# Ignalina/znippy

Measured on AMD Instinct MI355X. Metric: decompress MB/s (uncompressed) + compress MB/s, 100k x 10KB archive, higher is better.
Workload: dtype u8; 1 GPU; 100k x 10KiB text chunks (BASELINE configs[1]); rows_per_gpu=100000, chunk_bytes=10240, bytes_per_gpu=1024000000, blob_bytes_per_gpu=6400000, parallelism=row-cursor ranges x1, pipelining=step k+1 queued before step k's counters are read (two runs in flight)

## Files before the change

znippy_amd/csrc/api.hip:

```cpp
#include <unistd.h>
#include "common.h"
#include "encode.h"
#include "../../include/znippy_hip.h"

#include <algorithm>
#include <cstdio>
#include <cstdlib>
#include <cstring>
#include <chrono>
#include <memory>
#include <new>
#include <stdexcept>
#include <string>
#include <vector>
#include <unordered_map>

namespace zn {
int measure_b3_pass_ns(int cus, hipStream_t s, float *ns_per_pass_per_simd, float *ghz);
size_t decode_lit_scratch_bytes(int grid);
void set_fused_dbg(unsigned long long *p);
void set_fused_abl(int v);
}

using namespace zn;
// ... 63 lines not shown
    uint64_t bx_fse_cap = 0, bx_huf_cap = 0;
    uint32_t *rx_pool = nullptr, *rx_chunk = nullptr;
    uint8_t *rx_cdone = nullptr;
    uint64_t rx_cap = 0;
    uint8_t *vs_pool = nullptr;
    uint64_t vs_cap = 0;
    uint8_t *rr_pool[2] = {nullptr, nullptr};
    uint64_t rr_cap[2] = {0, 0};
    hipEvent_t ev_fork = nullptr, ev_join = nullptr, ev_join2 = nullptr;
    std::vector<KTime> ktimes;
    int n_ktimes = 0;
    std::vector<hipEvent_t> event_pool;
    bool ktime_open = false;
    std::vector<std::pair<size_t, void *>> pinned_pool;
    size_t pinned_pool_bytes = 0;
    std::vector<std::pair<size_t, void *>> dev_pool;
    std::unordered_map<void *, size_t> dev_sizes;
    size_t dev_pool_bytes = 0;
    struct {
        int dbg = 0;
        unsigned lds_pad = 0;
        int store_g = 0;
        bool no_block_items = false, no_fused_blocks = false, ddbg = false, edbg = false, no_fused_store = false,
             nohash = false, no_roles = false, no_fz = false, fz_only = false, no_bx = false, tdbg = false, no_fuse_hash = false, trace = false, no_rx = false, no_pack = false, no_lean = false, no_stored_only = false;
        unsigned roles_min = 2048;
        unsigned bx_big = BX_BIG_SEQ;
        bool bx_big_set = false;
        int ktime = 2;
    } sw;
    int cus = 256;
    int live_tables = 0;
    bool closing = false;
    unsigned long long *clk_buf = nullptr;
    enum Diag { DIAG_FUSED, DIAG_ITEMS, DIAG_FZ, DIAG_GENERAL, DIAG_BX, DIAG_ENCODE, DIAG_N };
    unsigned long long *diag[DIAG_N] = {};
};

static void read_switches(znippy_ctx *ctx) {
    auto on = [](const char *n) { const char *v = getenv(n); return v && *v && *v != '0'; };
    if (const char *e = getenv("ZNIPPY_DBG")) ctx->sw.dbg = atoi(e);
    if (const char *e = getenv("ZNIPPY_LDS_PAD")) ctx->sw.lds_pad = (unsigned)atoi(e);
    ctx->sw.no_block_items = on("ZNIPPY_NO_BLOCK_ITEMS");
    ctx->sw.no_fused_blocks = on("ZNIPPY_NO_FUSED_BLOCKS");
    ctx->sw.ddbg = on("ZNIPPY_DDBG");
    ctx->sw.edbg = on("ZNIPPY_EDBG");
    ctx->sw.no_fused_store = on("ZNIPPY_NO_FUSED_STORE");
    ctx->sw.nohash = on("ZNIPPY_NOHASH");
    ctx->sw.no_roles = on("ZNIPPY_NO_ROLES");
    ctx->sw.no_fz = on("ZNIPPY_NO_FZ");
    ctx->sw.tdbg = on("ZNIPPY_TDBG");
    ctx->sw.trace = on("ZNIPPY_TRACE");
    ctx->sw.no_lean = on("ZNIPPY_NO_LEAN");
    ctx->sw.no_pack = on("ZNIPPY_NO_PACK");
    if (const char *e = getenv("ZNIPPY_STORE_G")) ctx->sw.store_g = atoi(e) == 1 ? 1 : (atoi(e) == 2 ? 2 : 0);
    ctx->sw.no_stored_only = on("ZNIPPY_NO_STORED_ONLY");
    ctx->sw.no_rx = on("ZNIPPY_NO_RX");
    ctx->sw.no_fuse_hash = on("ZNIPPY_NO_FUSE_HASH");
    ctx->sw.no_bx = on("ZNIPPY_NO_BX");
    if (const char *e = getenv("ZNIPPY_BX_BIG")) { ctx->sw.bx_big = (unsigned)atoi(e); ctx->sw.bx_big_set = true; }
    if (const char *lv = getenv("ZNIPPY_LEVEL")) { const int v = atoi(lv); if (v >= 1 && v <= 22) ctx->level = v; }
    if (const char *wl = getenv("ZNIPPY_WINDOW_LOG")) { const int v = atoi(wl); if (v == 0 || (v >= WINDOW_LOG_MIN && v <= WINDOW_LOG_MAX)) ctx->window_log = v; }
    if (const char *gs = getenv("ZNIPPY_GEN_SHARE")) { const int v = atoi(gs); if (v >= 1 && v <= 4) ctx->gen_share = v; }
    ctx->sw.fz_only = on("ZNIPPY_FZ_ONLY");
    if (const char *e = getenv("ZNIPPY_ROLES_MIN")) ctx->sw.roles_min = (unsigned)atoi(e);
    if (const char *e = getenv("ZNIPPY_KTIME")) ctx->sw.ktime = atoi(e);
}

static void *pinned_take(znippy_ctx *ctx, size_t bytes, size_t *cap) {
    size_t best = ctx->pinned_pool.size();
    for (size_t i = 0; i < ctx->pinned_pool.size(); i++)
        if (ctx->pinned_pool[i].first >= bytes && ctx->pinned_pool[i].first <= 4 * bytes + 4096 &&
            (best == ctx->pinned_pool.size() || ctx->pinned_pool[i].first < ctx->pinned_pool[best].first))
            best = i;
    if (best != ctx->pinned_pool.size()) {
        void *p = ctx->pinned_pool[best].second;
// ... 187 lines not shown
static_assert(ctl_before(CTL_COUNTERS, CTL_HAND) && ctl_before(CTL_HAND, CTL_CURSORS) && ctl_before(CTL_CURSORS, CTL_FZ_POOL) && ctl_before(CTL_FZ_POOL, CTL_BX_POOL) &&
              ctl_before(CTL_BX_POOL, CTL_BX_CTR) && ctl_before(CTL_BX_CTR, CTL_RX) && CTL_RX.at + CTL_RX.bytes <= CTL_HEAD, "control block: regions overlap or pass the head");
static_assert(CTL_COUNTERS.at == 0 && CTL_HAND.at == CTL_COUNTERS.bytes && CTL_MIRROR == CTL_HAND.at + CTL_HAND.bytes, "the mirror is exactly counters + hand-over counts");
static_assert(CTL_FLAG < 8 && H_FLAGGED == H_SERIAL + 4 && H_FLAGGED < 8 && CUR_FZ_WORK < 16 && zn::RX_ROUNDS <= RX_ZERO && RX_ZERO < 16, "control block: a word outside its region");

struct znippy_rows {
    znippy_ctx *ctx = nullptr;
    uint64_t row_begin = 0;
    uint32_t n = 0;
    uint32_t n_compressed = 0;
    uint64_t *blob_off = nullptr, *blob_size = nullptr, *usize = nullptr, *out_off = nullptr;
    uint8_t *compressed = nullptr, *checksum = nullptr, *d_bitmap = nullptr;
    uint32_t *h_pack = nullptr, *d_pack = nullptr;
    size_t h_pack_cap = 0;
    unsigned long long *d_pack_sums = nullptr;
    uint8_t *ctl = nullptr;
    size_t ctl_bytes = 0;
    template <class T> T *ctl_at(CtlRegion g, size_t i = 0) const { return reinterpret_cast<T *>(ctl + g.at) + i; }
    uint32_t *hand(Hand h) const { return ctl_at<uint32_t>(CTL_HAND, h); }
    uint32_t *cur(Cursor c) const { return ctl_at<uint32_t>(CTL_CURSORS, c); }
    int32_t *status = nullptr;
    uint32_t *digests = nullptr;
    uint64_t *counters = nullptr;
    uint64_t *h_counters = nullptr;
    const uint32_t *mirror_hand(unsigned slot) const { return reinterpret_cast<const uint32_t *>(reinterpret_cast<const uint8_t *>(h_counters + 16 * slot) + CTL_HAND.at); }
    size_t h_counters_cap = 0;
    int bx_hint = -1;
    bool lean_ok = false;
    int lean_hint = -1;
    bool lean_blocks_ok = false;
    bool lean_mixed_ok = false;
    bool roles_off = false;
    bool small_ok = false, small_off = false;
    uint32_t *all_rows = nullptr;
    int lean_hint2 = -1;
    int plain_hint = -1;
    struct RunArgs { const void *blobs = nullptr; void *out = nullptr; uint64_t base = 0, cap = 0, blob_cap = ~0ull; bool verify = false, plain = false; } run_args[2];
    uint64_t *vs_off = nullptr;
    uint64_t vs_bytes = 0;
    bool vs_built = false;
    bool no_out = false;
    hipEvent_t ev_done[2] = {nullptr, nullptr};
    uint64_t run_seq = 0;
    uint64_t ext_min_bo = 0, ext_max_bend = 0, ext_max_oend = 0;
    bool ext_wrap = false;
    std::vector<uint64_t> h_blob_off, h_blob_size, h_len, h_out_off;
// ... 457 lines not shown
        ctx->own_stream = true;
    }
    init_fused_tables();
    if (hipStreamCreateWithFlags(&ctx->aux, hipStreamNonBlocking) != hipSuccess ||
        hipStreamCreateWithFlags(&ctx->copy, hipStreamNonBlocking) != hipSuccess ||
        hipEventCreateWithFlags(&ctx->ev_fork, hipEventDisableTiming) != hipSuccess ||
        hipEventCreateWithFlags(&ctx->ev_join, hipEventDisableTiming) != hipSuccess ||
        hipEventCreateWithFlags(&ctx->ev_join2, hipEventDisableTiming) != hipSuccess) {
        znippy_ctx_destroy(ctx);
        return ZNIPPY_E_HIP;
    }
    ctx->decode_grid = decode_grid_size(device);
    if (hipMalloc(&ctx->cursor, 64) != hipSuccess) {
        znippy_ctx_destroy(ctx);
        return ZNIPPY_E_NOMEM;
    }
    {
        hipDeviceProp_t p;
        int cus = hipGetDeviceProperties(&p, device) == hipSuccess ? p.multiProcessorCount : 256;
        ctx->cus = cus;
        ctx->encode_grid = cus * 8;
        ctx->encode_grid_small = cus * 16;
    }
    *out = ctx;
    return ZNIPPY_OK;
}

static void ctx_teardown(znippy_ctx *ctx);
void znippy_ctx_destroy(znippy_ctx *ctx) {
    if (!ctx || ctx->closing) return;
    if (ctx->live_tables) {
        (void)hipSetDevice(ctx->device);
        (void)hipStreamSynchronize(ctx->stream);
        ctx->closing = true;
        return;
    }
    ctx_teardown(ctx);
}
static void table_released(znippy_ctx *ctx) {
    if (--ctx->live_tables == 0 && ctx->closing) ctx_teardown(ctx);
}
static void ctx_teardown(znippy_ctx *ctx) {
    (void)hipSetDevice(ctx->device);
    (void)hipStreamSynchronize(ctx->stream);
    for (auto &k : ctx->ktimes) { (void)hipEventDestroy(k.t0); (void)hipEventDestroy(k.t1); }
    void *dev[] = {ctx->lit_scratch, ctx->lit_scratch_b, ctx->fz_lit_pool, ctx->fz_seq_pool, ctx->bx_fse_pool, ctx->bx_huf_pool, ctx->rx_pool, ctx->rx_chunk, ctx->rx_cdone, ctx->cursor, ctx->vs_pool, ctx->rr_pool[0], ctx->rr_pool[1],
                   ctx->clk_buf, ctx->shim_in, ctx->shim_out, ctx->enc_prov, ctx->enc_seq, ctx->enc_tabs, ctx->ldm};
    for (void *p : dev) if (p) (void)hipFree(p);
    for (unsigned long long *d : ctx->diag) if (d) (void)hipFree(d);
    if (ctx->aux) { (void)hipStreamSynchronize(ctx->aux); (void)hipStreamDestroy(ctx->aux); }
    if (ctx->copy) { (void)hipStreamSynchronize(ctx->copy); (void)hipStreamDestroy(ctx->copy); }
    for (auto &e : ctx->pinned_pool) (void)hipHostFree(e.second);
    for (auto &e : ctx->dev_pool) (void)hipFree(e.second);
    for (hipEvent_t e : ctx->event_pool) (void)hipEventDestroy(e);
    if (ctx->ev_fork) (void)hipEventDestroy(ctx->ev_fork);
    if (ctx->ev_join) (void)hipEventDestroy(ctx->ev_join);
    if (ctx->ev_join2) (void)hipEventDestroy(ctx->ev_join2);
    if (ctx->own_stream) (void)hipStreamDestroy(ctx->stream);
    delete ctx;
}

const char *znippy_last_error(const znippy_ctx *ctx) { return ctx ? ctx->err.c_str() : "null context"; }

int znippy_ctx_sync(znippy_ctx *ctx) {
    if (ctx && ctx->closing) return ZNIPPY_E_INVAL;
    if (!ctx) return ZNIPPY_E_INVAL;
    HIPCHK(ctx, hipStreamSynchronize(ctx->stream));
    if (ctx->copy) HIPCHK(ctx, hipStreamSynchronize(ctx->copy));
    return ZNIPPY_OK;
}

int znippy_last_kernel_times(znippy_ctx *ctx, const char **names, float *ms, int cap) {
    if (ctx && ctx->closing) return ZNIPPY_E_INVAL;
    if (!ctx) return 0;
    int n = std::min(cap, ctx->n_ktimes);
    for (int i = 0; i < n; i++) {
        names[i] = ctx->ktimes[i].name;
        ms[i] = 0.f;
        (void)hipEventElapsedTime(&ms[i], ctx->ktimes[i].t0, ctx->ktimes[i].t1);
    }
    return n;
}

int znippy_rows_foreign_stats(znippy_ctx *ctx, znippy_rows *r, uint64_t stats[8]) {
    if (ctx && ctx->closing) return ZNIPPY_E_INVAL;
    if (!ctx || !r || r->ctx != ctx || !stats) return ZNIPPY_E_INVAL;
    HIPCHK(ctx, hipSetDevice(ctx->device));
    HIPCHK(ctx, hipStreamSynchronize(ctx->stream));
    HIPCHK(ctx, hipMemcpy(stats, r->ctl + (r->bx_slots ? CTL_BX_POOL : CTL_FZ_POOL).at, 64, hipMemcpyDeviceToHost));
    return ZNIPPY_OK;
// ... 69 lines not shown
    if (n < 5) return ZNIPPY_E_CORRUPT;
    uint32_t magic;
    memcpy(&magic, p, 4);
    if (magic != 0xFD2FB528u) return ZNIPPY_E_CORRUPT;
    uint32_t fhd = p[4], fcs_flag = fhd >> 6, single = (fhd >> 5) & 1, did_flag = fhd & 3;
    if (fhd & 8) return ZNIPPY_E_CORRUPT;
    uint32_t fcs_bytes = fcs_flag == 0 ? single : (1u << fcs_flag);
    uint32_t did_bytes = did_flag == 3 ? 4 : did_flag;
    size_t pos = 5 + (single ? 0 : 1) + did_bytes;
    if (n < pos + fcs_bytes) return ZNIPPY_E_CORRUPT;
    if (!fcs_bytes) return ZNIPPY_E_UNSUPPORTED;
    uint64_t fcs = 0;
    for (uint32_t i = 0; i < fcs_bytes; i++) fcs |= (uint64_t)p[pos + i] << (8 * i);
    if (fcs_bytes == 2) fcs += 256;
    *out_size = fcs;
    return ZNIPPY_OK;
}


void znippy_rows_destroy(znippy_rows *r) {
    if (!r) return;
    (void)hipSetDevice(r->ctx->device);
    void *ptrs[] = {r->blob_off, r->blob_size, r->usize, r->out_off, r->compressed, r->checksum,
                    r->ctl, r->digests, r->corrupt, r->list_a, r->pending,
                    r->cand_row, r->cand_base, r->cand_nblocks, r->fz_base, r->fz_cap, r->fz_it_cand, r->fz_nb, r->fz_work, r->fz_items, r->item_row, r->item_k, r->item_src, r->row_flag, r->pending2,
                    r->bt_tile, r->bt_item, r->tile_done, r->todo, r->status_init, r->slow_list,
                    r->bx_cand_row, r->bx_cand_base, r->bx_cand_nb, r->bx_huf_list, r->bx_seq_list, r->bx_items, r->bx_prep, r->d_bitmap, r->bx_sort_tmp,
                    r->rx_base, r->rx_fail, r->rx_blk, r->rx_list, r->d_pack, r->d_pack_sums, r->all_rows, r->vs_off, r->tree_dev};
    for (void *p : ptrs)
        tfree(r->ctx, p);
    if (r->h_counters) {
        (void)hipStreamSynchronize(r->ctx->stream);
        pinned_give(r->ctx, r->h_counters, r->h_counters_cap);
    }
    if (r->h_pack) {
        (void)hipStreamSynchronize(r->ctx->stream);
        pinned_give(r->ctx, r->h_pack, r->h_pack_cap);
    }
    for (hipEvent_t e : r->ev_done) event_give(r->ctx, e);
    free_plan(r->ctx, r->plan);
    znippy_ctx *const c = r->ctx;
    delete r;
    table_released(c);
}

struct RowCols {
    const uint64_t *bo, *bs, *us, *oo;
    const uint8_t *bitmap;
    uint64_t row_begin, row_end;
    bool allc;
    uint32_t comp(uint32_t i) const { if (allc) return 1u; const uint64_t row = row_begin + i; return (bitmap[row >> 3] >> (row & 7)) & 1u; }
};
struct RowClasses {
    std::vector<uint32_t> la, cand_row, cand_base, cand_nb, item_row, item_k, fz_base, fz_cap, fz_it_cand;
    uint64_t big_bytes = 0, big_blob = 0, n_big = 0, nblk = 0;
};

static int rows_columns_h2d(znippy_ctx *ctx, znippy_rows *r, const RowCols &c, const uint8_t *checksum, TDbg &td) {
    const uint32_t n = r->n;
    int rc = ZNIPPY_OK;
    const uint64_t bm0 = c.row_begin >> 3, bm1 = (c.row_end + 7) >> 3;
    bool packed = false;
// ... 154 lines not shown
    ctx->live_tables++;
    r->row_begin = row_begin;
    r->n = (uint32_t)(row_end - row_begin);
    const uint32_t n = r->n;
    bool allc = true;
    if (compressed_bitmap) {
        uint64_t row = row_begin;
        for (; row < row_end && (row & 7); row++) allc &= (compressed_bitmap[row >> 3] >> (row & 7)) & 1;
        for (; row + 8 <= row_end && allc; row += 8) allc &= compressed_bitmap[row >> 3] == 0xFF;
        for (; row < row_end && allc; row++) allc &= (compressed_bitmap[row >> 3] >> (row & 7)) & 1;
    }
    std::vector<uint64_t> own_oo;
    if (!out_offset) {
        r->no_out = true;
        own_oo.resize(n);
        uint64_t at = 0;
        for (uint32_t i = 0; i < n; i++) { own_oo[i] = at; at += uncompressed_size[row_begin + i]; }
    }
    const RowCols c{blob_offset + row_begin, blob_size + row_begin, uncompressed_size + row_begin, out_offset ? out_offset + row_begin : own_oo.data(), compressed_bitmap, row_begin, row_end, allc};
    int rc = rows_columns_h2d(ctx, r, c, checksum, td);
    if (rc) return rc;
    r->corrupt_cap = std::max<uint32_t>(n, 1);
    r->ctl_bytes = CTL_HEAD + std::max<size_t>(4 * (size_t)n, 16);
    if (tmalloc(ctx, &r->ctl, r->ctl_bytes) != hipSuccess ||
        tmalloc(ctx, &r->digests, std::max<size_t>(32 * (size_t)n, 32)) != hipSuccess ||
        !(r->h_counters = (uint64_t *)pinned_take(ctx, 256, &r->h_counters_cap)) ||
        !(r->ev_done[0] = event_take(ctx)) || !(r->ev_done[1] = event_take(ctx)) ||
        tmalloc(ctx, &r->corrupt, 8 * (size_t)r->corrupt_cap) != hipSuccess)
        return ZNIPPY_E_NOMEM;
    r->counters = r->ctl_at<uint64_t>(CTL_COUNTERS);
    r->status = reinterpret_cast<int32_t *>(r->ctl + CTL_HEAD);
    td.mark("allocs");
    PlanBuf p;
    build_plan([=, us = c.us, bs = c.bs, &c](uint32_t i) -> uint64_t { return (allc || c.comp(i)) ? us[i] : bs[i]; }, n, p);
    td.mark("plan");
    if ((rc = upload_plan(ctx, p, r->plan))) return rc;
    td.mark("plan_h2d");
    for (const Tile &t : p.tiles) r->n_small_tiles += t.n_units != 0;
    if (r->n_small_tiles && tmalloc(ctx, &r->slow_list, 4 * (size_t)p.tiles.size()) != hipSuccess) return ZNIPPY_E_NOMEM;
    RowClasses k;
    rows_classify(ctx, r, c, k);
    r->n_list_a = (uint32_t)k.la.size();
    td.mark("big_rows");
    if (r->n_compressed && (rc = rows_batch_buffers(ctx, r, k.nblk))) return rc;
    r->wide_rows = k.n_big && k.big_bytes / k.n_big >= (1u << 20) && k.big_blob * 50 < k.big_bytes;
    r->n_cand = (uint32_t)k.cand_row.size();
    r->n_items = (uint32_t)k.item_row.size();
    const bool hints = !ctx->sw.no_lean && r->n_list_a == 0;
    const uint32_t n_tiles = (uint32_t)p.tiles.size();
    r->small_ok = allc && hints && !ctx->sw.no_bx && r->n_cand == 0 && r->n_small_tiles == n_tiles && r->n_small_tiles > 0 && r->bx_slots;
    r->lean_mixed_ok = hints && r->n_cand == 0 && r->n_small_tiles > 0 && r->n_small_tiles < n_tiles;
    r->lean_blocks_ok = allc && hints && r->n_cand > 0 && r->n_small_tiles == 0;
    r->lean_ok = allc && hints && r->n_cand == 0 && p.big.empty() && r->n_small_tiles == n_tiles && r->n_small_tiles > 0;
    if (r->n_cand && (rc = rows_item_buffers(ctx, r, k))) return rc;
// ... 161 lines not shown
    a.list_a = r->list_a; a.n_list_a = r->n_list_a;
    a.pending = r->pending; a.pending_count = r->hand(H_FUSED);
    a.compressed = r->compressed;
    a.n_rows = r->n; a.cursor = r->cur(CUR_GENERAL);
    a.lit_scratch = ctx->lit_scratch;
    if (ctx->sw.ddbg)
        a.dbg = diag_cycle<8>(ctx, znippy_ctx::DIAG_GENERAL, ctx->stream, nullptr, [](const unsigned long long *h) {
            if (h[0]) fprintf(stderr, "[znippy ddbg] general decoder frames=%llu  kcycles per frame: headers+tree=%.1f huffman-table=%.1f literal-streams=%.1f seq-tables=%.1f first-batch=%.1f decode+execute=%.1f tail=%.1f\n", h[0],
                              h[6] / 1e3 / h[0], h[7] / 1e3 / h[0], h[1] / 1e3 / h[0], h[2] / 1e3 / h[0], h[3] / 1e3 / h[0], h[4] / 1e3 / h[0], h[5] / 1e3 / h[0]);
        });
    return a;
}
static void decode_rest(znippy_ctx *ctx, const znippy_rows *r, DecodeArgs a, uint32_t rows) {
    a.list_a = nullptr; a.n_list_a = 0;
    a.pending = r->pending2; a.pending_count = r->hand(H_SERIAL);
    a.cursor = r->cur(CUR_FALLBACK);
    timed(ctx, "zstd_decode_fallback", ctx->stream, [&] {
        if (!ctx->sw.fz_only) launch_decode(a, std::min<int>(ctx->decode_grid, (int)rows), r->wide_rows, ctx->stream);
    });
}

static int run_clear(znippy_ctx *ctx, znippy_rows *r, const RunPlan &p, const RowsRun &run) {
    hipStream_t s = ctx->stream;
    if (run.preset) HIPCHK(ctx, hipMemcpyAsync(r->ctl, r->status_init, r->ctl_bytes, hipMemcpyDeviceToDevice, s));
    else HIPCHK(ctx, hipMemsetAsync(r->ctl, 0, r->ctl_bytes, s));
    if (p.small_off) HIPCHK(ctx, hipMemsetD32Async((hipDeviceptr_t)r->hand(H_FUSED), (int)r->n, 1, s));
    return ZNIPPY_OK;
}

static int run_small_rows(znippy_ctx *ctx, znippy_rows *r, const RunPlan &p, const RowsRun &run) {
    hipStream_t s = ctx->stream;
    FusedArgs f{};
    f.h = rows_hash_args(ctx, r, run);
    f.h.pass = 1;
    f.blob_size = r->blob_size; f.out_cap = run.out_cap; f.status = r->status;
    f.preset = run.preset;
    f.pending = r->pending; f.pending_count = r->hand(H_FUSED);
    if (run.plain) {
        if (r->n_small_tiles) timed(ctx, "decode_small", s, [&] { launch_decode_small(f, s); });
        return ZNIPPY_OK;
    }
    f.dbg = ctx->sw.dbg;
    if (f.dbg & 8) {
        f.dbg_buf = diag_cycle<8>(ctx, znippy_ctx::DIAG_FUSED, s, nullptr, [](const unsigned long long *h4) {
            if (h4[3]) fprintf(stderr, "[znippy dbg] waves=%llu prologue=%.0f decode=%.0f hash=%.0f | parse+lits=%.0f expand-build=%.0f stream-out=%.0f after-match=%.0f cycles/wave\n", h4[3],
                               (double)h4[0] / h4[3], (double)h4[1] / h4[3], (double)h4[2] / h4[3], (double)h4[6] / h4[3], (double)h4[4] / h4[3], (double)h4[5] / h4[3], (double)h4[7] / h4[3]);
// ... 215 lines not shown

static void run_second_hash(znippy_ctx *ctx, znippy_rows *r, const RunPlan &p, const RowsRun &run) {
    hipStream_t s = ctx->stream;
    HashArgs h = rows_hash_args(ctx, r, run);
    h.pass = p.stored_only ? 0 : 2;
    h.tile_done = r->n_bt && !p.stored_only ? r->tile_done : nullptr;
    timed(ctx, run.verify ? "blake3_hash_only" : "blake3_second_pass", s, [&] { launch_hash_tiles(h, s); });
    if (r->plan.n_big)
        timed(ctx, "blake3_merge_big", s, [&] {
            launch_merge_big(r->plan.big, r->plan.n_big, r->plan.tile_cv, r->digests, r->plan.grp_big, r->plan.grp_k, r->plan.n_grp, r->plan.max_cvs, s);
        });
}

static void run_copy_stored(znippy_ctx *ctx, znippy_rows *r, const RunPlan &p, const RowsRun &run) {
    if (!p.stored_only && !r->plan.n_big) return;
    const HashArgs h = rows_hash_args(ctx, r, run);
    timed(ctx, "copy_stored", ctx->stream, [&] { launch_copy_stored(h, p.stored_only, ctx->stream); });
}

static int run_verify(znippy_ctx *ctx, znippy_rows *r, const RunPlan &p, const RowsRun &run) {
    hipStream_t s = ctx->stream;
    if (p.lean_mixed) HIPCHK(ctx, hipStreamWaitEvent(s, ctx->ev_join, 0));
    const bool skipped = p.lean || p.lean_blocks || p.lean_mixed;
    timed(ctx, run.plain ? "count_rows" : "verify", s, [&] {
        launch_verify(r->digests, run.plain ? nullptr : r->checksum, r->usize, r->status, r->n, r->row_begin, r->counters, r->corrupt, r->corrupt_cap, s,
                      skipped ? r->ctl_at<uint32_t>(CTL_HAND) : nullptr, (p.lean || p.lean_mixed) ? LEAN_SMALL : LEAN_BLOCKS);
    });
    HIPCHK(ctx, hipMemcpyAsync(r->h_counters + 16 * run.slot, r->counters, CTL_MIRROR, hipMemcpyDeviceToHost, s));
    HIPCHK(ctx, hipEventRecord(r->ev_done[run.slot], s));
    HIPCHK(ctx, hipGetLastError());
    return ZNIPPY_OK;
}

static int rows_launch(znippy_ctx *ctx, znippy_rows *r, const void *d_blobs, uint64_t blob_base, void *d_out, uint64_t out_cap,
                       unsigned slot, bool verify, bool plain, bool *queued = nullptr) {
    ctx->n_ktimes = 0;
    int rc = ensure_decoder(ctx);
    if (!rc && verify) {
        rc = rows_verify_slots(ctx, r);
        if (!rc) rc = ensure_verify_scratch(ctx, r->vs_bytes);
        d_out = ctx->vs_pool; out_cap = r->vs_bytes;
    }
    if (!rc) rc = rows_validate(ctx, r, blob_base, out_cap, verify);
    if (!rc && r->fz_total) rc = ensure_fz_pools(ctx, r->fz_bytes, r->fz_total);
    if (!rc && r->bx_slots) {
        rc = ensure_fz_pools(ctx, r->bx_bytes, r->bx_item_cap);
        if (!rc) rc = ensure_bx_pools(ctx, r->bx_bytes, r->bx_item_cap);
        if (!rc && r->rx_base && rows_route_hint(r, plain) != 0) rc = ensure_rx_pool(ctx, r->rx_words);
    }
    if (rc) return rc;
    if (r->n_cand && !ctx->lit_scratch_b && hipMalloc(&ctx->lit_scratch_b, decode_lit_scratch_bytes(ctx->decode_grid)) != hipSuccess) return ZNIPPY_E_NOMEM;
    if (r->run_seq && rows_route_hint(r, plain) < 0 && r->n) {
        const unsigned last = (unsigned)((r->run_seq - 1) & 1);
        const bool last_plain = r->run_args[last].plain;
        if (last_plain && !plain) (void)0;
        else if (hipEventQuery(r->ev_done[last]) != hipSuccess) (void)hipGetLastError();
        else if (last_plain) rows_note_plain(r, last);
        else rows_note_hint(r, last);
    }
    const RowsRun run{d_blobs, blob_base, d_out, out_cap, r->n_bad ? 1 : 0, slot, verify, plain};
    const RunPlan p = rows_plan(ctx, r, run.preset, plain);
    if (p.small_off && !r->all_rows) {
        if (tmalloc(ctx, &r->all_rows, 4 * (size_t)r->n) != hipSuccess) return ZNIPPY_E_NOMEM;
        hipLaunchKernelGGL(k_iota32, dim3((r->n + 255) / 256), dim3(256), 0, ctx->stream, r->all_rows, r->n);
    }
    { auto &ra = r->run_args[slot]; ra.blobs = d_blobs; ra.base = blob_base; ra.out = verify ? nullptr : d_out; ra.cap = verify ? 0 : out_cap; ra.blob_cap = r->blob_cap; ra.verify = verify; ra.plain = plain; }
    if (queued) *queued = true;
    if ((rc = run_clear(ctx, r, p, run)) || !r->n) return rc;
    if (!p.small_off && !p.stored_only && (rc = run_small_rows(ctx, r, p, run))) return rc;
    if (p.decode && r->n_cand && (rc = run_block_items(ctx, r, p, run))) return rc;
    if (p.decode && r->n_compressed && (rc = p.bx ? run_batch_path(ctx, r, p, run) : run_serial_flow(ctx, r, p, run))) return rc;
    if (plain) run_copy_stored(ctx, r, p, run);
    else if (!p.lean) run_second_hash(ctx, r, p, run);
    return run_verify(ctx, r, p, run);
}

static void rows_abandon(znippy_ctx *ctx, znippy_rows *r);
static int rows_queue(znippy_ctx *ctx, znippy_rows *r, const void *d_blobs, uint64_t blob_base, void *d_out, uint64_t out_cap, bool verify, bool plain = false) {
    HIPCHK(ctx, hipSetDevice(ctx->device));
    bool queued = false;
    const int rc = rows_launch(ctx, r, d_blobs, blob_base, d_out, out_cap, (unsigned)(r->run_seq & 1), verify, plain, &queued);
    if (rc && queued) rows_abandon(ctx, r);
    if (rc) return rc;
    r->run_seq++;
    return ZNIPPY_OK;
}
static void rows_abandon(znippy_ctx *ctx, znippy_rows *r) {
    if (hipEventRecord(ctx->ev_join, ctx->aux) == hipSuccess) (void)hipStreamWaitEvent(ctx->stream, ctx->ev_join, 0);
    (void)hipStreamSynchronize(ctx->stream);
// ... 33 lines not shown
    HIPCHK(ctx, hipSetDevice(ctx->device));
    int rc = rows_verify_slots(ctx, r);
    if (!rc) rc = ensure_verify_scratch(ctx, r->vs_bytes);
    if (rc) return rc;
    *d_base = r->vs_bytes ? ctx->vs_pool : nullptr;
    *bytes = r->vs_bytes;
    if (row_offset && r->n) {
        std::vector<uint8_t> comp(r->n);
        std::vector<uint64_t> len(r->n);
        HIPCHK(ctx, hipStreamSynchronize(ctx->stream));
        HIPCHK(ctx, hipMemcpy(row_offset, r->vs_off, 8 * (size_t)r->n, hipMemcpyDeviceToHost));
        HIPCHK(ctx, hipMemcpy(comp.data(), r->compressed, r->n, hipMemcpyDeviceToHost));
        HIPCHK(ctx, hipMemcpy(len.data(), r->usize, 8 * (size_t)r->n, hipMemcpyDeviceToHost));
        for (uint32_t i = 0; i < r->n; i++)
            if (!comp[i] || !len[i]) row_offset[i] = ~0ull;
    }
    return ZNIPPY_OK;
}

static int rows_settle(znippy_ctx *ctx, znippy_rows *r, unsigned slot) {
    if (!r->n || !r->run_seq || !(r->h_counters[16 * slot + 7])) return ZNIPPY_OK;
    HIPCHK(ctx, hipSetDevice(ctx->device));
    HIPCHK(ctx, hipStreamSynchronize(ctx->stream));
    r->force_full = true;
    r->lean_hint = 0; r->lean_hint2 = 0;
    const unsigned latest = (unsigned)((r->run_seq - 1) & 1);
    const unsigned order[2] = {slot, latest};
    for (int i = 0; i < (slot == latest ? 1 : 2); i++) {
        const znippy_rows::RunArgs ra = r->run_args[order[i]];
        r->blob_cap = ra.blob_cap;
        bool queued = false;
        const int rc = rows_launch(ctx, r, ra.blobs, ra.base, ra.out, ra.cap, order[i], ra.verify, ra.plain, &queued);
        if (rc) {
            if (queued) rows_abandon(ctx, r);
            return rc;
        }
    }
    HIPCHK(ctx, hipStreamSynchronize(ctx->stream));
    return ZNIPPY_OK;
}

int znippy_rows_results_lagged(znippy_ctx *ctx, znippy_rows *r, unsigned lag, znippy_verify_counters *counters) {
    if (ctx && ctx->closing) return ZNIPPY_E_INVAL;
    if (!ctx || !r || r->ctx != ctx || !counters || lag > 1 || r->run_seq <= lag) return ZNIPPY_E_INVAL;
    uint64_t c[8] = {0};
    if (r->n) {
        const unsigned slot = (unsigned)((r->run_seq - 1 - lag) & 1);
        HIPCHK(ctx, hipEventSynchronize(r->ev_done[slot]));
        { const int rc = rows_settle(ctx, r, slot); if (rc) return rc; }
        memcpy(c, r->h_counters + 16 * slot, 64);
        if (r->run_args[slot].plain) rows_note_plain(r, slot);
        else rows_note_hint(r, slot);
    }
    counters->total_chunks = c[0]; counters->total_written_bytes = c[1]; counters->verified_bytes = c[2];
    counters->corrupt_bytes = c[3]; counters->corrupt_rows = c[4]; counters->decode_errors = c[5];
    return ZNIPPY_OK;
}

int znippy_rows_results(znippy_ctx *ctx, znippy_rows *r, znippy_verify_counters *counters,
                        uint64_t *corrupt_rows, uint64_t corrupt_cap, int32_t *row_status) {
    if (ctx && ctx->closing) return ZNIPPY_E_INVAL;
    if (!ctx || !r) return ZNIPPY_E_INVAL;
    HIPCHK(ctx, hipSetDevice(ctx->device));
    HIPCHK(ctx, hipStreamSynchronize(ctx->stream));
    uint64_t c[8] = {0};
    if (r->n && r->run_seq) {
        { const int rc = rows_settle(ctx, r, (unsigned)((r->run_seq - 1) & 1)); if (rc) return rc; }
        memcpy(c, r->h_counters + 16 * ((r->run_seq - 1) & 1), 64);
        if (r->run_args[(r->run_seq - 1) & 1].plain) rows_note_plain(r, (unsigned)((r->run_seq - 1) & 1));
        else rows_note_hint(r, (unsigned)((r->run_seq - 1) & 1));
    }
    if (counters) {
        counters->total_chunks = c[0]; counters->total_written_bytes = c[1]; counters->verified_bytes = c[2];
        counters->corrupt_bytes = c[3]; counters->corrupt_rows = c[4]; counters->decode_errors = c[5];
    }
    if (corrupt_rows && corrupt_cap && c[4]) {
        uint64_t k = std::min<uint64_t>(c[4], r->corrupt_cap);
        std::vector<uint64_t> tmp(k);
        HIPCHK(ctx, hipMemcpy(tmp.data(), r->corrupt, 8 * k, hipMemcpyDeviceToHost));
        std::sort(tmp.begin(), tmp.end());
        memcpy(corrupt_rows, tmp.data(), 8 * std::min<uint64_t>(k, corrupt_cap));
    }
    if (row_status && r->n) {
        HIPCHK(ctx, hipMemcpy(row_status, r->status, 4 * (size_t)r->n, hipMemcpyDeviceToHost));
        for (uint32_t i = 0; i < r->n; i++)
            if (row_status[i] > 0) row_status[i] = 0;
    }
// ... 551 lines not shown
            if (!ok[i] && row_status) row_status[sel[i]] = ZNIPPY_E_DIGEST;
        }
    }
    HIPCHK(ctx, hipStreamSynchronize(s));
    std::swap(r->tree_dev, g.tree);
    r->tree_accept.swap(accept);
    return ZNIPPY_OK;
}

#define ZN_NO_THROW(call) \
    try { return call; } catch (const std::bad_alloc &) { return ZNIPPY_E_NOMEM; } catch (const std::length_error &) { return ZNIPPY_E_NOMEM; }
int znippy_rows_block_tree_layout(znippy_ctx *ctx, znippy_rows *r, uint64_t *n_entries, uint64_t *row_first) { ZN_NO_THROW(rows_block_tree_layout(ctx, r, n_entries, row_first)) }
int znippy_rows_block_tree_build(znippy_ctx *ctx, znippy_rows *r, const void *d_blobs, uint64_t blob_base, uint8_t *tree, int32_t *row_status) {
    ZN_NO_THROW(rows_block_tree_build(ctx, r, d_blobs, blob_base, tree, row_status))
}
int znippy_rows_set_block_tree(znippy_ctx *ctx, znippy_rows *r, const uint8_t *tree, int32_t *row_status) { ZN_NO_THROW(rows_set_block_tree(ctx, r, tree, row_status)) }
#undef ZN_NO_THROW

int znippy_rows_digests(znippy_ctx *ctx, znippy_rows *r, uint8_t *digests) {
    if (ctx && ctx->closing) return ZNIPPY_E_INVAL;
    if (!ctx || !r || !digests) return ZNIPPY_E_INVAL;
    HIPCHK(ctx, hipSetDevice(ctx->device));
    HIPCHK(ctx, hipStreamSynchronize(ctx->stream));
    if (r->n && r->run_seq) { const int rc = rows_settle(ctx, r, (unsigned)((r->run_seq - 1) & 1)); if (rc) return rc; }
    if (r->run_seq && r->run_args[(r->run_seq - 1) & 1].plain) return ZNIPPY_E_INVAL;
    if (r->n) HIPCHK(ctx, hipMemcpy(digests, r->digests, 32 * (size_t)r->n, hipMemcpyDeviceToHost));
    return ZNIPPY_OK;
}

static void rounds_select(znippy_rounds *r, unsigned slot) {
    const size_t n = r->n;
    r->res = r->res_m[slot];
    r->h_res = r->h_res_m[slot];
    r->total = reinterpret_cast<uint64_t *>(r->res);
    r->overflow = reinterpret_cast<uint32_t *>(r->res + 8);
    r->blob_offset = reinterpret_cast<uint64_t *>(r->res + 16);
    r->blob_size = r->blob_offset + n;
    r->digests = reinterpret_cast<uint32_t *>(r->res + 16 + n * 16);
}

void znippy_rounds_destroy(znippy_rounds *r) {
    if (!r) return;
    (void)hipSetDevice(r->ctx->device);
    if (r->ctx->copy) (void)hipStreamSynchronize(r->ctx->copy);
    for (int k = 0; k < 2; k++) {
        pinned_give(r->ctx, r->h_res_m[k], r->h_res_cap_m[k]);
// ... 495 lines not shown
```

znippy_amd/csrc/common.h:

```cpp
#pragma once
#include <hip/hip_runtime.h>
#include <stdint.h>
#include <stddef.h>

namespace zn {

struct Tile {
    uint32_t first_unit;
    uint32_t n_units;
    uint32_t first_leaf;
    uint32_t n_leaves;
    uint32_t cv_index;
    uint32_t pad;
};

struct BigUnit {
    uint32_t unit;
    uint32_t cv_base;
    uint32_t n_cvs;
    uint32_t pad;
};

struct HashArgs {
    const Tile *tiles;
// ... 66 lines not shown
    HashArgs h;
    const uint64_t *blob_size;
    const uint32_t *bt_tile, *bt_item;
    uint32_t n_bt;
    const uint32_t *item_src;
    const uint32_t *row_flag;
    uint8_t *tile_done, *item_done;
    int dbg;
};
void launch_fused_blocks(const FusedBlocksArgs &a, hipStream_t s, bool verify = false);

void launch_hash_tiles(const HashArgs &a, hipStream_t s);
void launch_fused_small(const FusedArgs &a, hipStream_t s, int grid_cap = 0, bool verify = false);
void launch_fused_roles(const FusedArgs &a, int cus, hipStream_t s, bool verify = false);
void init_fused_tables();
void launch_decode_small(const FusedArgs &a, hipStream_t s);
void launch_decode_blocks(const FusedBlocksArgs &a, hipStream_t s);
void launch_copy_stored(const HashArgs &a, bool all, hipStream_t s);
void launch_merge_big(const BigUnit *big, uint32_t n_big, uint32_t *tile_cv, uint32_t *digests, const uint32_t *grp_big,
                      const uint32_t *grp_k, uint32_t n_grp, uint32_t max_cvs, hipStream_t s);
void launch_verify(const uint32_t *digests, const uint8_t *checksum, const uint64_t *usize,
                   const int32_t *status, uint32_t n_rows, uint64_t row_begin, uint64_t *counters,
                   uint64_t *corrupt_rows, uint32_t corrupt_cap, hipStream_t s, const uint32_t *lean_lists = nullptr, uint32_t lean_mask = 0);
int decode_grid_size(int device);
void launch_decode(const DecodeArgs &a, int grid, bool wide, hipStream_t s);
struct BlockScanArgs {
    const uint32_t *cand_row, *cand_base, *cand_nblocks;
    uint32_t n_cand;
    const uint8_t *blobs;
    uint64_t blob_base;
    const uint64_t *blob_off, *blob_size, *usize, *out_off;
    uint64_t out_cap;
    uint32_t *item_src;
    uint32_t *row_flag;
    int32_t *status;
    uint32_t *pending, *pending_count;
    int preset;
};
void launch_scan_blocks(const BlockScanArgs &a, hipStream_t s);
void launch_compact_items(const uint8_t *item_done, uint32_t n_items, uint32_t *todo, uint32_t *n_todo, hipStream_t s);
void launch_finish_blocks(const BlockScanArgs &a, hipStream_t s, bool defer_flagged);

struct FzItem {
    uint32_t src;
    uint32_t out;
    uint32_t nseq;
// ... 120 lines not shown
```

znippy_amd/csrc/fused_small.hip:

```cpp
#include "common.h"
#include "hash_dev.h"

#include <algorithm>
#include <cstring>

namespace zn {

constexpr uint32_t EOFF_MAX = 960;
constexpr uint32_t EBUF = EOFF_MAX + 1024 + 64;
constexpr int F_E_CORRUPT = -5, F_E_UNSUP = -6, F_E_DST = -4;
constexpr int F_NOT_SIMPLE = 1;

struct DTab {
    uint16_t next;
    uint8_t nbits, addbits;
    uint32_t base;
};
__constant__ DTab c_dll[64], c_dml[64], c_dof[32];
__constant__ uint32_t c_llb[36] = {0, 1, 2, 3, 4, 5, 6, 7, 8, 9, 10, 11, 12, 13, 14, 15, 16, 18,
                                   20, 22, 24, 28, 32, 40, 48, 64, 128, 256, 512, 1024, 2048,
                                   4096, 8192, 16384, 32768, 65536};
__constant__ uint8_t c_lla[36] = {0, 0, 0, 0, 0, 0, 0, 0, 0, 0, 0, 0, 0, 0, 0, 0, 1, 1,
                                  1, 1, 2, 2, 3, 3, 4, 6, 7, 8, 9, 10, 11, 12, 13, 14, 15, 16};
__constant__ uint32_t c_mlb[53] = {3, 4, 5, 6, 7, 8, 9, 10, 11, 12, 13, 14, 15, 16, 17, 18, 19, 20,
// ... 1386 lines not shown
    if (threadIdx.x < 64 * R_LOADERS) {
        if (!(a.dbg & 64)) __builtin_amdgcn_s_setprio(3);
        roles_loader<STORE>(a, S);
    } else roles_hasher<STORE>(a, S);
    if (clk) { a.dbg_buf[0] = __builtin_amdgcn_s_memtime() - c0; a.dbg_buf[1] = __builtin_amdgcn_s_memrealtime() - r0; }
}

void launch_fused_roles(const FusedArgs &a, int cus, hipStream_t s, bool verify) {
    if (!a.h.n_tiles) return;
    static bool attr_set[2] = {false, false};
    if (!attr_set[verify]) {
        (void)hipFuncSetAttribute(verify ? reinterpret_cast<const void *>(k_fused_roles<false>) : reinterpret_cast<const void *>(k_fused_roles<true>),
                                  hipFuncAttributeMaxDynamicSharedMemorySize, (int)sizeof(RolesShared));
        attr_set[verify] = true;
    }
    const uint32_t want = (a.h.n_tiles + R_GROUP - 1) / R_GROUP;
    const uint32_t per_cu = sizeof(RolesShared) > 80 * 1024 ? 1u : 2u;
    uint32_t grid = std::min<uint32_t>((uint32_t)cus * per_cu, want);
    if (a.lds_pad) grid = std::min<uint32_t>(grid, a.lds_pad);
    if (verify) hipLaunchKernelGGL(k_fused_roles<false>, dim3(grid), dim3(R_WAVES * 64), sizeof(RolesShared), s, a);
    else hipLaunchKernelGGL(k_fused_roles<true>, dim3(grid), dim3(R_WAVES * 64), sizeof(RolesShared), s, a);
}

template <bool STORE>
__global__ __launch_bounds__(256, 4) void k_fused_blocks(FusedBlocksArgs a) {
    __shared__ __attribute__((aligned(16))) uint8_t s_area[4][STAGE_FULL_BYTES];
    uint32_t *const s_nodes = reinterpret_cast<uint32_t *>(&s_area[0][0]);
    constexpr uint32_t AREA_NODES = STAGE_FULL_BYTES / 32;
    static_assert(STAGE_FULL_BYTES % 32 == 0, "area must be a whole number of nodes");
    __shared__ uint32_t s_tab[3][4 * FOLD_UNITS];
    __shared__ __attribute__((aligned(16))) uint8_t s_Wb[4][WSTRIDE];
    __shared__ uint16_t s_d[4][3];
    const uint32_t lane = threadIdx.x & 63, w = threadIdx.x >> 6;
    if (lane < FOLD_UNITS) s_tab[0][w * FOLD_UNITS + lane] = 0;
    const uint32_t idx = blockIdx.x * 4 + w;
    if (idx < a.n_bt) {
        const uint32_t ti = a.bt_tile[idx], item = a.bt_item[idx];
        const Tile t = a.h.tiles[ti];
        const uint32_t row = t.first_unit;
        const uint32_t src_pos = a.item_src[item];
        const uint64_t usize = a.h.len[row];
        const uint64_t origin = (uint64_t)(t.first_leaf >> 7) << 17;
        if (src_pos != 0xFFFFFFFFu && a.row_flag[row] == 0 && t.n_leaves == 64 && usize - origin >= 128 * 1024) {
            uint8_t *const WL = s_Wb[w];
            const uint64_t n = a.blob_size[row];
            const uint8_t *const src = a.h.srcA + (a.h.offA[row] - a.h.baseA) + src_pos;
// ... 241 lines not shown
```

znippy_amd/csrc/hash_kernels.hip:

```cpp
#include "common.h"
#include "hash_dev.h"

namespace zn {

typedef __attribute__((address_space(3))) uint32_t lds_u32;
template <int G>
__device__ __noinline__ void fold_first_level(lds_u32 *nodes) {
    const uint32_t lane = threadIdx.x & 63;
    const bool on = lane < 32 * G;
    const lds_u4a *c = reinterpret_cast<const lds_u4a *>(nodes + (size_t)(2 * lane) * 8);
    u4v l0 = u4v{0, 0, 0, 0}, l1 = l0, r0 = l0, r1 = l0;
    if (on) { l0 = c[0]; l1 = c[1]; r0 = c[2]; r1 = c[3]; }
    uint32_t L[8] = {l0.x, l0.y, l0.z, l0.w, l1.x, l1.y, l1.z, l1.w}, R[8] = {r0.x, r0.y, r0.z, r0.w, r1.x, r1.y, r1.z, r1.w}, cv[8];
    b3::parent(cv, L, R, false);
    __builtin_amdgcn_wave_barrier();
    if (on) {
        lds_u4a *d = reinterpret_cast<lds_u4a *>(nodes + (size_t)lane * 8);
        d[0] = u4v{cv[0], cv[1], cv[2], cv[3]};
        d[1] = u4v{cv[4], cv[5], cv[6], cv[7]};
    }
}
template <int G>
__device__ __noinline__ void fold_wg_tiles(lds_u32 *base, uint32_t area_nodes, uint32_t *tile_cv, uint32_t cvi) {
    constexpr uint32_t NT = 4 * G;
// ... 247 lines not shown
    }
}

void launch_merge_big(const BigUnit *big, uint32_t n_big, uint32_t *tile_cv, uint32_t *digests, const uint32_t *grp_big,
                      const uint32_t *grp_k, uint32_t n_grp, uint32_t max_cvs, hipStream_t s) {
    if (!n_big) return;
    if (n_grp && max_cvs <= MERGE_UNIT_MAX_CVS) {
        hipLaunchKernelGGL(k_merge_units, dim3(n_big), dim3(64 * MERGE_UNIT_WAVES), 0, s, big, n_big, tile_cv, digests);
        return;
    }
    if (n_grp) hipLaunchKernelGGL(k_merge_groups, dim3(n_grp), dim3(64), 0, s, big, grp_big, grp_k, n_grp, tile_cv);
    hipLaunchKernelGGL(k_merge_big, dim3(n_big), dim3(64), 0, s, big, n_big, tile_cv, digests);
}

__global__ __launch_bounds__(256) void k_verify(const uint32_t *digests, const uint8_t *checksum,
                                                const uint64_t *usize, const int32_t *status, uint32_t n_rows,
                                                uint64_t row_begin, unsigned long long *counters,
                                                uint64_t *corrupt_rows, uint32_t corrupt_cap, const uint32_t *lean_lists, uint32_t lean_mask) {
    if (lean_lists && blockIdx.x == 0 && threadIdx.x == 0) {
        uint32_t any = 0;
        for (uint32_t i = 0; i < 8; i++) if ((lean_mask >> i) & 1u) any |= lean_lists[i];
        if (any) counters[7] = 1;
    }
    unsigned long long v[6] = {0, 0, 0, 0, 0, 0};
    for (uint32_t r = blockIdx.x * 256 + threadIdx.x; r < n_rows; r += gridDim.x * 256) {
        v[0] += 1;
        if (status && status[r] < 0) {
            v[5] += 1;
        } else {
            const unsigned long long len = usize[r];
            v[1] += len;
            bool ok = true;
            if (checksum) {
                const uint4 *want = reinterpret_cast<const uint4 *>(checksum) + (size_t)r * 2;
                const uint4 *got = reinterpret_cast<const uint4 *>(digests) + (size_t)r * 2;
                const uint4 w0 = want[0], w1 = want[1], g0 = got[0], g1 = got[1];
                ok = w0.x == g0.x && w0.y == g0.y && w0.z == g0.z && w0.w == g0.w &&
                     w1.x == g1.x && w1.y == g1.y && w1.z == g1.z && w1.w == g1.w;
            }
            if (ok) v[2] += len;
            else {
                v[3] += len;
                v[4] += 1;
                unsigned long long slot = atomicAdd(&counters[6], 1ull);
                if (corrupt_rows && slot < corrupt_cap) corrupt_rows[slot] = row_begin + r;
            }
        }
    }
    __shared__ unsigned long long red[6][4];
#pragma unroll
    for (int c = 0; c < 6; c++) {
        unsigned long long x = v[c];
#pragma unroll
        for (int d = 32; d >= 1; d >>= 1) x += __shfl_xor(x, d);
        if ((threadIdx.x & 63) == 0) red[c][threadIdx.x >> 6] = x;
    }
    __syncthreads();
    if (threadIdx.x < 6) {
        unsigned long long x = red[threadIdx.x][0] + red[threadIdx.x][1] + red[threadIdx.x][2] + red[threadIdx.x][3];
        if (x) atomicAdd(&counters[threadIdx.x], x);
    }
}

void launch_verify(const uint32_t *digests, const uint8_t *checksum, const uint64_t *usize,
                   const int32_t *status, uint32_t n_rows, uint64_t row_begin, uint64_t *counters,
                   uint64_t *corrupt_rows, uint32_t corrupt_cap, hipStream_t s, const uint32_t *lean_lists, uint32_t lean_mask) {
    if (!n_rows) return;
    hipLaunchKernelGGL(k_verify, dim3(std::min<uint32_t>((n_rows + 255) / 256, 128)), dim3(256), 0, s, digests, checksum, usize, status,
                       n_rows, row_begin, reinterpret_cast<unsigned long long *>(counters), corrupt_rows, corrupt_cap, lean_lists, lean_mask);
}

__global__ __launch_bounds__(256) void k_b3_pass_ubench(uint32_t *out, uint32_t seed, int passes, unsigned long long *clk) {
    const unsigned long long c0 = __builtin_amdgcn_s_memtime(), r0 = __builtin_amdgcn_s_memrealtime();
    uint32_t cv[8], m[16];
#pragma unroll
    for (int i = 0; i < 8; i++) cv[i] = threadIdx.x * 7 + i + seed;
#pragma unroll
    for (int i = 0; i < 16; i++) m[i] = threadIdx.x * 13 + i * seed;
#pragma unroll 1
    for (int p = 0; p < passes; p++) {
        b3::compress(cv, m, (uint32_t)p, 0, 64, 0);
        m[p & 15] ^= cv[0];
    }
    uint32_t x = 0;
#pragma unroll
    for (int i = 0; i < 8; i++) x ^= cv[i];
    out[blockIdx.x * 256 + threadIdx.x] = x;
    if (clk && blockIdx.x == 7 && threadIdx.x == 0) {
        clk[0] = __builtin_amdgcn_s_memtime() - c0;
        clk[1] = __builtin_amdgcn_s_memrealtime() - r0;
    }
}
// ... 31 lines not shown
```

Baseline: 1.953 million MB/s.

## Fork verify kernel onto aux stream with double-buffered control state

On the lean path, the verify kernel now runs on a secondary stream forked by an event, so it can overlap the next run's main-stream work. Control, digest and corrupt buffers are double-buffered per slot to make that safe, and sync points now also wait on the aux stream. Forking is enabled only when register and LDS footprint checks show verify can co-reside with the roles kernel. The verify kernel also keeps narrower counters and uses an XOR-OR digest compare to cut register use.

Result: faster. 1.996 million MB/s (median of 6 runs) (+2.2%).

```diff
diff --git a/znippy_amd/csrc/api.hip b/znippy_amd/csrc/api.hip
--- a/znippy_amd/csrc/api.hip
+++ b/znippy_amd/csrc/api.hip
@@ -109,13 +109,14 @@
         unsigned lds_pad = 0;
         int store_g = 0;
         bool no_block_items = false, no_fused_blocks = false, ddbg = false, edbg = false, no_fused_store = false,
-             nohash = false, no_roles = false, no_fz = false, fz_only = false, no_bx = false, tdbg = false, no_fuse_hash = false, trace = false, no_rx = false, no_pack = false, no_lean = false, no_stored_only = false;
+             no_fork_verify = false, nohash = false, no_roles = false, no_fz = false, fz_only = false, no_bx = false, tdbg = false, no_fuse_hash = false, trace = false, no_rx = false, no_pack = false, no_lean = false, no_stored_only = false;
         unsigned roles_min = 2048;
         unsigned bx_big = BX_BIG_SEQ;
         bool bx_big_set = false;
         int ktime = 2;
     } sw;
     int cus = 256;
+    bool fork_verify = false;
     int live_tables = 0;
     bool closing = false;
     unsigned long long *clk_buf = nullptr;
@@ -138,6 +139,7 @@
     ctx->sw.tdbg = on("ZNIPPY_TDBG");
     ctx->sw.trace = on("ZNIPPY_TRACE");
     ctx->sw.no_lean = on("ZNIPPY_NO_LEAN");
+    ctx->sw.no_fork_verify = on("ZNIPPY_NO_FORK_VERIFY");
     ctx->sw.no_pack = on("ZNIPPY_NO_PACK");
     if (const char *e = getenv("ZNIPPY_STORE_G")) ctx->sw.store_g = atoi(e) == 1 ? 1 : (atoi(e) == 2 ? 2 : 0);
     ctx->sw.no_stored_only = on("ZNIPPY_NO_STORED_ONLY");
@@ -371,6 +373,16 @@
     int32_t *status = nullptr;
     uint32_t *digests = nullptr;
     uint64_t *counters = nullptr;
+    uint8_t *ctl_m[2] = {nullptr, nullptr};
+    uint32_t *digests_m[2] = {nullptr, nullptr};
+    uint64_t *corrupt_m[2] = {nullptr, nullptr};
+    void select(unsigned slot) {
+        ctl = ctl_m[slot]; digests = digests_m[slot]; corrupt = corrupt_m[slot];
+        counters = ctl_at<uint64_t>(CTL_COUNTERS);
+        status = reinterpret_cast<int32_t *>(ctl + CTL_HEAD);
+    }
+    hipEvent_t ev_main[2] = {nullptr, nullptr};
+    bool aux_used = false;
     uint64_t *h_counters = nullptr;
     const uint32_t *mirror_hand(unsigned slot) const { return reinterpret_cast<const uint32_t *>(reinterpret_cast<const uint8_t *>(h_counters + 16 * slot) + CTL_HAND.at); }
     size_t h_counters_cap = 0;
@@ -874,6 +886,11 @@
         ctx->encode_grid = cus * 8;
         ctx->encode_grid_small = cus * 16;
     }
+    if (!ctx->sw.no_fork_verify) {
+        int rr = 0, rw = 0, rl = 0, vr = 0, vl = 0;
+        if (roles_footprint(&rr, &rw, &rl) == 0 && verify_footprint(&vr, &vl) == 0)
+            ctx->fork_verify = rw * ((rr + 7) / 8 * 8) + (vr + 7) / 8 * 8 <= 512 && rl + vl <= 160 * 1024 && rw + 1 <= 8;
+    }
     *out = ctx;
     return ZNIPPY_OK;
 }
@@ -884,6 +901,7 @@
     if (ctx->live_tables) {
         (void)hipSetDevice(ctx->device);
         (void)hipStreamSynchronize(ctx->stream);
+        if (ctx->aux) (void)hipStreamSynchronize(ctx->aux);
         ctx->closing = true;
         return;
     }
@@ -895,6 +913,7 @@
 static void ctx_teardown(znippy_ctx *ctx) {
     (void)hipSetDevice(ctx->device);
     (void)hipStreamSynchronize(ctx->stream);
+    if (ctx->aux) (void)hipStreamSynchronize(ctx->aux);
     for (auto &k : ctx->ktimes) { (void)hipEventDestroy(k.t0); (void)hipEventDestroy(k.t1); }
     void *dev[] = {ctx->lit_scratch, ctx->lit_scratch_b, ctx->fz_lit_pool, ctx->fz_seq_pool, ctx->bx_fse_pool, ctx->bx_huf_pool, ctx->rx_pool, ctx->rx_chunk, ctx->rx_cdone, ctx->cursor, ctx->vs_pool, ctx->rr_pool[0], ctx->rr_pool[1],
                    ctx->clk_buf, ctx->shim_in, ctx->shim_out, ctx->enc_prov, ctx->enc_seq, ctx->enc_tabs, ctx->ldm};
@@ -918,6 +937,7 @@
     if (ctx && ctx->closing) return ZNIPPY_E_INVAL;
     if (!ctx) return ZNIPPY_E_INVAL;
     HIPCHK(ctx, hipStreamSynchronize(ctx->stream));
+    if (ctx->aux) HIPCHK(ctx, hipStreamSynchronize(ctx->aux));
     if (ctx->copy) HIPCHK(ctx, hipStreamSynchronize(ctx->copy));
     return ZNIPPY_OK;
 }
@@ -1033,11 +1053,12 @@
     if (!r) return;
     (void)hipSetDevice(r->ctx->device);
     void *ptrs[] = {r->blob_off, r->blob_size, r->usize, r->out_off, r->compressed, r->checksum,
-                    r->ctl, r->digests, r->corrupt, r->list_a, r->pending,
+                    r->ctl_m[0], r->ctl_m[1], r->digests_m[0], r->digests_m[1], r->corrupt_m[0], r->corrupt_m[1], r->list_a, r->pending,
                     r->cand_row, r->cand_base, r->cand_nblocks, r->fz_base, r->fz_cap, r->fz_it_cand, r->fz_nb, r->fz_work, r->fz_items, r->item_row, r->item_k, r->item_src, r->row_flag, r->pending2,
                     r->bt_tile, r->bt_item, r->tile_done, r->todo, r->status_init, r->slow_list,
                     r->bx_cand_row, r->bx_cand_base, r->bx_cand_nb, r->bx_huf_list, r->bx_seq_list, r->bx_items, r->bx_prep, r->d_bitmap, r->bx_sort_tmp,
                     r->rx_base, r->rx_fail, r->rx_blk, r->rx_list, r->d_pack, r->d_pack_sums, r->all_rows, r->vs_off, r->tree_dev};
+    if (r->aux_used && hipEventRecord(r->ctx->ev_join, r->ctx->aux) == hipSuccess) (void)hipStreamWaitEvent(r->ctx->stream, r->ctx->ev_join, 0);
     for (void *p : ptrs)
         tfree(r->ctx, p);
     if (r->h_counters) {
@@ -1049,6 +1070,7 @@
         pinned_give(r->ctx, r->h_pack, r->h_pack_cap);
     }
     for (hipEvent_t e : r->ev_done) event_give(r->ctx, e);
+    for (hipEvent_t e : r->ev_main) event_give(r->ctx, e);
     free_plan(r->ctx, r->plan);
     znippy_ctx *const c = r->ctx;
     delete r;
@@ -1249,14 +1271,14 @@
     if (rc) return rc;
     r->corrupt_cap = std::max<uint32_t>(n, 1);
     r->ctl_bytes = CTL_HEAD + std::max<size_t>(4 * (size_t)n, 16);
-    if (tmalloc(ctx, &r->ctl, r->ctl_bytes) != hipSuccess ||
-        tmalloc(ctx, &r->digests, std::max<size_t>(32 * (size_t)n, 32)) != hipSuccess ||
-        !(r->h_counters = (uint64_t *)pinned_take(ctx, 256, &r->h_counters_cap)) ||
-        !(r->ev_done[0] = event_take(ctx)) || !(r->ev_done[1] = event_take(ctx)) ||
-        tmalloc(ctx, &r->corrupt, 8 * (size_t)r->corrupt_cap) != hipSuccess)
-        return ZNIPPY_E_NOMEM;
-    r->counters = r->ctl_at<uint64_t>(CTL_COUNTERS);
-    r->status = reinterpret_cast<int32_t *>(r->ctl + CTL_HEAD);
+    for (int s = 0; s < 2; s++)
+        if (tmalloc(ctx, &r->ctl_m[s], r->ctl_bytes) != hipSuccess ||
+            tmalloc(ctx, &r->digests_m[s], std::max<size_t>(32 * (size_t)n, 32)) != hipSuccess ||
+            tmalloc(ctx, &r->corrupt_m[s], 8 * (size_t)r->corrupt_cap) != hipSuccess ||
+            !(r->ev_done[s] = event_take(ctx)) || !(r->ev_main[s] = event_take(ctx)))
+            return ZNIPPY_E_NOMEM;
+    if (!(r->h_counters = (uint64_t *)pinned_take(ctx, 256, &r->h_counters_cap))) return ZNIPPY_E_NOMEM;
+    r->select(0);
     td.mark("allocs");
     PlanBuf p;
     build_plan([=, us = c.us, bs = c.bs, &c](uint32_t i) -> uint64_t { return (allc || c.comp(i)) ? us[i] : bs[i]; }, n, p);
@@ -1464,6 +1486,7 @@
 
 static int run_clear(znippy_ctx *ctx, znippy_rows *r, const RunPlan &p, const RowsRun &run) {
     hipStream_t s = ctx->stream;
+    if (r->aux_used) HIPCHK(ctx, hipStreamWaitEvent(s, r->ev_done[run.slot], 0));
     if (run.preset) HIPCHK(ctx, hipMemcpyAsync(r->ctl, r->status_init, r->ctl_bytes, hipMemcpyDeviceToDevice, s));
     else HIPCHK(ctx, hipMemsetAsync(r->ctl, 0, r->ctl_bytes, s));
     if (p.small_off) HIPCHK(ctx, hipMemsetD32Async((hipDeviceptr_t)r->hand(H_FUSED), (int)r->n, 1, s));
@@ -1725,6 +1748,12 @@
     hipStream_t s = ctx->stream;
     if (p.lean_mixed) HIPCHK(ctx, hipStreamWaitEvent(s, ctx->ev_join, 0));
     const bool skipped = p.lean || p.lean_blocks || p.lean_mixed;
+    if (ctx->fork_verify && p.lean) {
+        HIPCHK(ctx, hipEventRecord(r->ev_main[run.slot], s));
+        s = ctx->aux;
+        HIPCHK(ctx, hipStreamWaitEvent(s, r->ev_main[run.slot], 0));
+        r->aux_used = true;
+    }
     timed(ctx, run.plain ? "count_rows" : "verify", s, [&] {
         launch_verify(r->digests, run.plain ? nullptr : r->checksum, r->usize, r->status, r->n, r->row_begin, r->counters, r->corrupt, r->corrupt_cap, s,
                       skipped ? r->ctl_at<uint32_t>(CTL_HAND) : nullptr, (p.lean || p.lean_mixed) ? LEAN_SMALL : LEAN_BLOCKS);
@@ -1768,6 +1797,7 @@
         hipLaunchKernelGGL(k_iota32, dim3((r->n + 255) / 256), dim3(256), 0, ctx->stream, r->all_rows, r->n);
     }
     { auto &ra = r->run_args[slot]; ra.blobs = d_blobs; ra.base = blob_base; ra.out = verify ? nullptr : d_out; ra.cap = verify ? 0 : out_cap; ra.blob_cap = r->blob_cap; ra.verify = verify; ra.plain = plain; }
+    r->select(slot);
     if (queued) *queued = true;
     if ((rc = run_clear(ctx, r, p, run)) || !r->n) return rc;
     if (!p.small_off && !p.stored_only && (rc = run_small_rows(ctx, r, p, run))) return rc;
@@ -1847,6 +1877,7 @@
     if (!r->n || !r->run_seq || !(r->h_counters[16 * slot + 7])) return ZNIPPY_OK;
     HIPCHK(ctx, hipSetDevice(ctx->device));
     HIPCHK(ctx, hipStreamSynchronize(ctx->stream));
+    HIPCHK(ctx, hipStreamSynchronize(ctx->aux));
     r->force_full = true;
     r->lean_hint = 0; r->lean_hint2 = 0;
     const unsigned latest = (unsigned)((r->run_seq - 1) & 1);
@@ -1888,6 +1919,7 @@
     if (!ctx || !r) return ZNIPPY_E_INVAL;
     HIPCHK(ctx, hipSetDevice(ctx->device));
     HIPCHK(ctx, hipStreamSynchronize(ctx->stream));
+    if (r->aux_used) HIPCHK(ctx, hipStreamSynchronize(ctx->aux));
     uint64_t c[8] = {0};
     if (r->n && r->run_seq) {
         { const int rc = rows_settle(ctx, r, (unsigned)((r->run_seq - 1) & 1)); if (rc) return rc; }
@@ -2485,6 +2517,7 @@
     if (!ctx || !r || !digests) return ZNIPPY_E_INVAL;
     HIPCHK(ctx, hipSetDevice(ctx->device));
     HIPCHK(ctx, hipStreamSynchronize(ctx->stream));
+    if (r->aux_used) HIPCHK(ctx, hipStreamSynchronize(ctx->aux));
     if (r->n && r->run_seq) { const int rc = rows_settle(ctx, r, (unsigned)((r->run_seq - 1) & 1)); if (rc) return rc; }
     if (r->run_seq && r->run_args[(r->run_seq - 1) & 1].plain) return ZNIPPY_E_INVAL;
     if (r->n) HIPCHK(ctx, hipMemcpy(digests, r->digests, 32 * (size_t)r->n, hipMemcpyDeviceToHost));
diff --git a/znippy_amd/csrc/common.h b/znippy_amd/csrc/common.h
--- a/znippy_amd/csrc/common.h
+++ b/znippy_amd/csrc/common.h
@@ -112,6 +112,8 @@
 void launch_verify(const uint32_t *digests, const uint8_t *checksum, const uint64_t *usize,
                    const int32_t *status, uint32_t n_rows, uint64_t row_begin, uint64_t *counters,
                    uint64_t *corrupt_rows, uint32_t corrupt_cap, hipStream_t s, const uint32_t *lean_lists = nullptr, uint32_t lean_mask = 0);
+int verify_footprint(int *regs, int *lds);
+int roles_footprint(int *regs, int *waves_per_simd, int *lds);
 int decode_grid_size(int device);
 void launch_decode(const DecodeArgs &a, int grid, bool wide, hipStream_t s);
 struct BlockScanArgs {
diff --git a/znippy_amd/csrc/fused_small.hip b/znippy_amd/csrc/fused_small.hip
--- a/znippy_amd/csrc/fused_small.hip
+++ b/znippy_amd/csrc/fused_small.hip
@@ -1432,6 +1432,14 @@
     else hipLaunchKernelGGL(k_fused_roles<true>, dim3(grid), dim3(R_WAVES * 64), sizeof(RolesShared), s, a);
 }
 
+int roles_footprint(int *regs, int *waves_per_simd, int *lds) {
+    hipFuncAttributes fa;
+    if (hipFuncGetAttributes(&fa, reinterpret_cast<const void *>(k_fused_roles<true>)) != hipSuccess) { (void)hipGetLastError(); return -1; }
+    const int per_cu = sizeof(RolesShared) > 80 * 1024 ? 1 : 2;
+    *regs = fa.numRegs; *waves_per_simd = (int)(R_WAVES * per_cu + 3) / 4; *lds = per_cu * (int)(sizeof(RolesShared) + fa.sharedSizeBytes);
+    return 0;
+}
+
 template <bool STORE>
 __global__ __launch_bounds__(256, 4) void k_fused_blocks(FusedBlocksArgs a) {
     __shared__ __attribute__((aligned(16))) uint8_t s_area[4][STAGE_FULL_BYTES];
diff --git a/znippy_amd/csrc/hash_kernels.hip b/znippy_amd/csrc/hash_kernels.hip
--- a/znippy_amd/csrc/hash_kernels.hip
+++ b/znippy_amd/csrc/hash_kernels.hip
@@ -293,31 +293,34 @@
         for (uint32_t i = 0; i < 8; i++) if ((lean_mask >> i) & 1u) any |= lean_lists[i];
         if (any) counters[7] = 1;
     }
-    unsigned long long v[6] = {0, 0, 0, 0, 0, 0};
+    uint32_t n_all = 0, n_bad = 0, n_err = 0;
+    unsigned long long ok_bytes = 0, bad_bytes = 0;
     for (uint32_t r = blockIdx.x * 256 + threadIdx.x; r < n_rows; r += gridDim.x * 256) {
-        v[0] += 1;
+        n_all += 1;
         if (status && status[r] < 0) {
-            v[5] += 1;
+            n_err += 1;
         } else {
             const unsigned long long len = usize[r];
-            v[1] += len;
             bool ok = true;
             if (checksum) {
                 const uint4 *want = reinterpret_cast<const uint4 *>(checksum) + (size_t)r * 2;
                 const uint4 *got = reinterpret_cast<const uint4 *>(digests) + (size_t)r * 2;
-                const uint4 w0 = want[0], w1 = want[1], g0 = got[0], g1 = got[1];
-                ok = w0.x == g0.x && w0.y == g0.y && w0.z == g0.z && w0.w == g0.w &&
-                     w1.x == g1.x && w1.y == g1.y && w1.z == g1.z && w1.w == g1.w;
+                uint4 w = want[0], g = got[0];
+                uint32_t d = (w.x ^ g.x) | (w.y ^ g.y) | (w.z ^ g.z) | (w.w ^ g.w);
+                w = want[1]; g = got[1];
+                d |= (w.x ^ g.x) | (w.y ^ g.y) | (w.z ^ g.z) | (w.w ^ g.w);
+                ok = d == 0;
             }
-            if (ok) v[2] += len;
+            if (ok) ok_bytes += len;
             else {
-                v[3] += len;
-                v[4] += 1;
+                bad_bytes += len;
+                n_bad += 1;
                 unsigned long long slot = atomicAdd(&counters[6], 1ull);
                 if (corrupt_rows && slot < corrupt_cap) corrupt_rows[slot] = row_begin + r;
             }
         }
     }
+    const unsigned long long v[6] = {n_all, ok_bytes + bad_bytes, ok_bytes, bad_bytes, n_bad, n_err};
     __shared__ unsigned long long red[6][4];
 #pragma unroll
     for (int c = 0; c < 6; c++) {
@@ -339,6 +342,13 @@
     if (!n_rows) return;
     hipLaunchKernelGGL(k_verify, dim3(std::min<uint32_t>((n_rows + 255) / 256, 128)), dim3(256), 0, s, digests, checksum, usize, status,
                        n_rows, row_begin, reinterpret_cast<unsigned long long *>(counters), corrupt_rows, corrupt_cap, lean_lists, lean_mask);
+}
+
+int verify_footprint(int *regs, int *lds) {
+    hipFuncAttributes fa;
+    if (hipFuncGetAttributes(&fa, reinterpret_cast<const void *>(k_verify)) != hipSuccess) { (void)hipGetLastError(); return -1; }
+    *regs = fa.numRegs; *lds = (int)fa.sharedSizeBytes;
+    return 0;
 }
 
 __global__ __launch_bounds__(256) void k_b3_pass_ubench(uint32_t *out, uint32_t seed, int passes, unsigned long long *clk) {
```
